# lazzati-astro/MCRaT

Measured on AMD Instinct MI355X. Metric: photon-scatter-events/sec at 1e6 photons, 2D FLASH jet, higher is better.
Workload: dtype f64

## Files before the change

mcrat_amd/csrc/frame_queue.hpp:

```cpp
#pragma once
#include <stddef.h>
#include <string.h>
#include "device_types.hpp"

#if defined(__HIPCC__)
#define MCRAT_FQ_HD __host__ __device__
#else
#define MCRAT_FQ_HD
#endif

namespace mcrat {

struct FrameItem {
    unsigned long long seed;
    double time_now;
    double remaining_time;
    double frame_end;
    int open;
    int hydro;
};
struct alignas(32) FrameRecord {
    double remaining_time, time_now;
    long long iterations;
    int done;
    int last_scattered_index;
    double last_time_step, last_scattered_temp;
    long long frame_scatt_cnt, n_relocated;
    long long not_found, kn_rejections, rescans, slot_steps;
    MCRAT_FQ_HD void from_state(const LoopState &s)
    {
        remaining_time = s.remaining_time; time_now = s.time_now; iterations = s.iterations; done = s.done; last_scattered_index = s.last_scattered_index;
        last_time_step = s.last_time_step; last_scattered_temp = s.last_scattered_temp; frame_scatt_cnt = s.frame_scatt_cnt; n_relocated = s.n_relocated;
        not_found = s.not_found; kn_rejections = s.kn_rejections; rescans = s.rescans; slot_steps = s.slot_steps;
    }
};
static_assert(sizeof(FrameRecord) <= 128, "the frame record stays compact: at most half a LoopState");
struct FrameQueueDev {
    int n_frames;
    int restore;
    int chain_clock;
    int pad;
    unsigned *ticket;
    const int *order;
    int order_off[9];
    unsigned *frames_done;
    const FrameItem *items;
    const HydroDev *hydro;
    FrameRecord *records;
    long long snap_delta;
    long long capture_delta, capture_stride;
};
constexpr unsigned FRAME_STALLED = 0x80000000u;
constexpr int FRAME_QUEUE_XCDS = 8, FRAME_TICKET_STRIDE = 16;


struct FrameQueueLayout {
    struct Range { size_t off, bytes; };
    size_t off_items, off_hydro, off_desc, off_ticket, off_done, off_rec, bytes;
    Range up;
    Range down;
    Range words;
    static size_t align_up(size_t x, size_t a) { return (x + a - 1) / a * a; }
    FrameQueueLayout(int R, int F, size_t n_hydro)
    {
        const size_t N = (size_t)R * (size_t)F;
        off_items = align_up(sizeof(int) * N, 64);
        off_hydro = align_up(off_items + sizeof(FrameItem) * N, 256);
        off_desc = align_up(off_hydro + sizeof(HydroDev) * n_hydro, 64);
        off_ticket = align_up(off_desc + sizeof(RankDesc) * (size_t)R, 256);
        off_done = off_ticket + sizeof(unsigned) * FRAME_QUEUE_XCDS * FRAME_TICKET_STRIDE;
        off_rec = align_up(off_done + sizeof(unsigned) * (size_t)R, 256);
        bytes = off_rec + sizeof(FrameRecord) * N;
        up = Range{0, off_rec};
        down = Range{off_ticket, bytes - off_ticket};
        words = Range{off_ticket, off_rec - off_ticket};
    }
    template <class T> static T *at(void *base, size_t off) { return reinterpret_cast<T *>(static_cast<char *>(base) + off); }
    int *order(void *b) const { return at<int>(b, 0); }
    FrameItem *items(void *b) const { return at<FrameItem>(b, off_items); }
    HydroDev *hydro(void *b) const { return at<HydroDev>(b, off_hydro); }
    RankDesc *desc(void *b) const { return at<RankDesc>(b, off_desc); }
    unsigned *ticket(void *b) const { return at<unsigned>(b, off_ticket); }
    unsigned *frames_done(void *b) const { return at<unsigned>(b, off_done); }
    FrameRecord *records(void *b) const { return at<FrameRecord>(b, off_rec); }
};

inline int frame_list_class(int r) { return r % FRAME_QUEUE_XCDS; }

inline int frame_queue_order(const FrameItem *items, int R, int F, const int *xcd_of_class, int *order, int *order_off)
{
    int count[FRAME_QUEUE_XCDS] = {0}, fill[FRAME_QUEUE_XCDS], n_open = 0, longest = 0;
    for (int f = 0; f < F; ++f)
        for (int r = 0; r < R; ++r)
            if (items[(size_t)f * R + r].open) count[xcd_of_class[frame_list_class(r)]] += 1;
    for (int x = 0; x < FRAME_QUEUE_XCDS; ++x) {
        order_off[x] = fill[x] = n_open;
        n_open += count[x];
        if (count[x] > longest) longest = count[x];
    }
    order_off[FRAME_QUEUE_XCDS] = n_open;
    for (int f = 0; f < F; ++f)
        for (int r = 0; r < R; ++r)
            if (items[(size_t)f * R + r].open) order[fill[xcd_of_class[frame_list_class(r)]]++] = f * R + r;
    return longest;
}
inline int frame_queue_groups(int longest_queue) { return FRAME_QUEUE_XCDS * longest_queue; }

enum FrameQueueNext { FRAME_QUEUE_DONE = 0, FRAME_QUEUE_GO_ON = 1, FRAME_QUEUE_NO_DRAW = 2 };
inline FrameQueueNext frame_queue_after_launch(unsigned *frames_done, unsigned *tickets, const FrameRecord *records, FrameItem *items, int R,
                                               const int *first, const int *last, bool chain_clock, int *stalled, int *xcd_of_class)
{
    bool all = true;
    for (int r = 0; r < R; ++r) {
        if (frames_done[r] & FRAME_STALLED) { frames_done[r] &= ~FRAME_STALLED; stalled[r] = (int)frames_done[r]; }
        all = all && (first[r] < 0 || (int)frames_done[r] == last[r] + 1);
    }
    if (all) return FRAME_QUEUE_DONE;
    int alive[FRAME_QUEUE_XCDS], n_alive = 0;
    for (int x = 0; x < FRAME_QUEUE_XCDS; ++x)
        if (tickets[(size_t)x * FRAME_TICKET_STRIDE] > 0) alive[n_alive++] = x;
    if (n_alive == 0) return FRAME_QUEUE_NO_DRAW;
    for (int k = 0; k < FRAME_QUEUE_XCDS; ++k)
        if (tickets[(size_t)xcd_of_class[k] * FRAME_TICKET_STRIDE] == 0) xcd_of_class[k] = alive[k % n_alive];
    memset(tickets, 0, sizeof(unsigned) * FRAME_QUEUE_XCDS * FRAME_TICKET_STRIDE);
    for (int r = 0; r < R; ++r) {
        if (first[r] < 0) continue;
        const int nf = (int)frames_done[r] > first[r] ? (int)frames_done[r] : first[r];
        for (int f = first[r]; f <= last[r]; ++f) {
            FrameItem &it = items[(size_t)f * R + r];
            if (f < nf) { it.open = 0; continue; }
            if (f > nf) continue;
            const FrameRecord &rec = records[(size_t)f * R + r];
            if (stalled[r] == nf && rec.iterations > 0 && !rec.done) it.open = 2;
            else if (chain_clock && f > first[r]) {
                it.time_now = records[(size_t)(f - 1) * R + r].time_now;
                it.remaining_time = it.frame_end - it.time_now;
// ... 8 lines not shown
```

mcrat_amd/csrc/kernels.hip:

```cpp
#include <hip/hip_runtime.h>
#include <limits.h>
#include <math.h>
#include <stdio.h>
#include <type_traits>
#include "device_types.hpp"
#include "launch.hpp"
#include "sc_exchange.hpp"
#include "physics.hpp"
#include "photon_cols.hpp"
#include "photon_plan.hpp"
#include "rng.hpp"
#include "cs_device.hpp"

#if !defined(MCRAT_TAU_TABLE_TU) || !defined(MCRAT_TU_DIMS)
#error "compile kernels.hip through kernels_d*.hip / kernels_table_d*.hip"
#endif
#define MCRAT_NS_CAT2(a, b) a##b
#define MCRAT_NS_CAT(a, b) MCRAT_NS_CAT2(a, b)
#if MCRAT_TAU_TABLE_TU
#define MCRAT_TU_NS MCRAT_NS_CAT(tau_table_d, MCRAT_TU_DIMS)
#else
#define MCRAT_TU_NS MCRAT_NS_CAT(tau_direct_d, MCRAT_TU_DIMS)
#endif

// ... 936 lines not shown
        if (nz && have + k == need - 1) *s_pos = q + 1;
        if (q >= n && have + k < need) *error = 1;
        __syncthreads();
        if (have + found >= need) { pos = *s_pos; have = need; }
        else { have += found; pos += BLOCK; }
        __syncthreads();
    }
    if (pos > n) { if (tid == 0) *error = 1; pos = n; }
    return pos;
}

__global__ __launch_bounds__(TAPE_BLOCK) void tape_draw_kernel(PhotonDev ph, const LoopState *__restrict__ st, TapeDev tape, Cand *__restrict__ block_min,
                                                                int n_blocks, Shortlist *sl)
{
    __shared__ double s_u[TAPE_BLOCK];
    __shared__ int s_w[TAPE_BLOCK / 64];
    __shared__ long long s_pos;
    __shared__ double s_wt[TAPE_BLOCK / 64];
    __shared__ int s_wi[TAPE_BLOCK / 64];
    if (st->done) return;
    const int tid = threadIdx.x;
    const double t_cut = st->t_cut;
    long long pos = *tape.cursor;
    if (tid == 0) sl->count = 0;
    __syncthreads();
    MinCand best;
    best.init();
    for (int c0 = 0; c0 < ph.n; c0 += TAPE_BLOCK) {
        const int i = c0 + tid;
        const bool valid = i < ph.n && (ph.flags[i] & FLAG_VALID);
        const bool located = valid && ph.idx[i] != -1;
        int need = 0;
        const int rank = block_exclusive_scan<TAPE_BLOCK>(located ? 1 : 0, s_w, need);
        pos = tape_take_nonzero<TAPE_BLOCK>(tape.u, tape.n, tape.error, pos, need, s_u, s_w, &s_pos);
        if (valid) {
            double t = ph.tts[i];
            if (located) {
                t = div_by_c(ph.ntau[i] * log(s_u[rank]));
                ph.tts[i] = t;
            }
            best.offer(t, i);
            if (t < t_cut) shortlist_push(sl, t, i);
        }
        __syncthreads();
    }
    wave_min_pair_dpp(best.t, best.i);
    if ((tid & 63) == 0) { s_wt[tid >> 6] = best.t; s_wi[tid >> 6] = best.i; }
    __syncthreads();
    if (tid == 0) {
        MinCand m;
        m.init();
        for (int w = 0; w < TAPE_BLOCK / 64; ++w) m.offer(s_wt[w], s_wi[w]);
        Cand c;
        c.t = m.t; c.idx = m.i; c.pad = 0;
        block_min[0] = c;
        *tape.cursor = pos;
    }
    for (int b = 1 + tid; b < n_blocks; b += TAPE_BLOCK) { Cand c; c.t = INFINITY; c.idx = INT_MAX; c.pad = 0; block_min[b] = c; }
}

__device__ __attribute__((noinline)) void copy_list_columns(double *r0, unsigned col_stride, int *idx, unsigned char *flags, char *type, int base, int n,
                                                            long long from, long long to, int tid, int block)
{
    for (int il = tid; il < n; il += block) {
        const size_t i = (size_t)base + il;
        double v[N_DOUBLE_COLS];
#pragma unroll
        for (int k = 0; k < N_DOUBLE_COLS; ++k)
            v[k] = *reinterpret_cast<const double *>(reinterpret_cast<const char *>(r0 + (size_t)k * col_stride + i) + from);
        const int ci = *reinterpret_cast<const int *>(reinterpret_cast<const char *>(idx + i) + from);
        const unsigned char cf = *reinterpret_cast<const unsigned char *>(reinterpret_cast<const char *>(flags + i) + from);
        const char ct = *(reinterpret_cast<const char *>(type + i) + from);
#pragma unroll
        for (int k = 0; k < N_DOUBLE_COLS; ++k)
            *reinterpret_cast<double *>(reinterpret_cast<char *>(r0 + (size_t)k * col_stride + i) + to) = v[k];
        *reinterpret_cast<int *>(reinterpret_cast<char *>(idx + i) + to) = ci;
        *reinterpret_cast<unsigned char *>(reinterpret_cast<char *>(flags + i) + to) = cf;
        *(reinterpret_cast<char *>(type + i) + to) = ct;
    }
}

template <unsigned MASK, int PITCH>
__device__ __attribute__((noinline)) void restore_list_columns_lds(double *r0, unsigned col_stride, int *idx, unsigned char *flags, char *type, int base,
                                                                   int n, long long from, unsigned char *lds, int tid, int block)
{
    using Cols = ListCols<MASK, PITCH>;
    static_assert((MASK & COLBIT_IDX) && (MASK & COLBIT_FLAGS), "idx and flags are among the LDS columns");
    typedef __attribute__((address_space(3))) unsigned char *LdsBytes;
    typedef __attribute__((address_space(3))) double *LdsDoubles;
    typedef __attribute__((address_space(3))) int *LdsInts;
    const LdsBytes l = (LdsBytes)lds;
    for (int il = tid; il < n; il += block) {
        const size_t i = (size_t)base + il;
        double v[N_DOUBLE_COLS];
#pragma unroll
        for (int k = 0; k < N_DOUBLE_COLS; ++k)
            v[k] = *reinterpret_cast<const double *>(reinterpret_cast<const char *>(r0 + (size_t)k * col_stride + i) + from);
        const int ci = *reinterpret_cast<const int *>(reinterpret_cast<const char *>(idx + i) + from);
        const unsigned char cf = *reinterpret_cast<const unsigned char *>(reinterpret_cast<const char *>(flags + i) + from);
        const char ct = *(reinterpret_cast<const char *>(type + i) + from);
#pragma unroll
        for (int k = 0; k < N_DOUBLE_COLS; ++k) {
            if (Cols::in_lds(k)) ((LdsDoubles)l)[Cols::lds_pos(k) * PITCH + il] = v[k];
            else r0[(size_t)k * col_stride + i] = v[k];
        }
        ((LdsInts)(l + Cols::lds_idx_bytes))[il] = ci;
        (l + Cols::lds_flags_bytes)[il] = cf;
        type[i] = ct;
    }
}

struct RankLayout {
    int n_ranks;
    int stride;
    int n_total;
    const RankDesc *desc;
    CsFrame *cs;
    const CsHookArgs *hook;
    FrameQueueDev fq;
};
struct TapeLayout : RankLayout {
    const double *tape_u;
    TapeList *tapes;
};
template <int BLOCK>
struct TapeLds {
    double u[BLOCK];
    int w[BLOCK / 64];
    long long pos, cursor;
};

#ifndef RANK_WAVES_PER_SIMD
#define RANK_WAVES_PER_SIMD 2
#endif
#ifndef RANK_NS_FUSED
#define RANK_NS_FUSED 2
#endif
#ifndef RANK_FUSE_DEN
#define RANK_FUSE_DEN 2
#endif

template <int DIMS, int GEOM, bool STOKES, bool RESIDENT, int RANK_BLOCK, bool FUSE, bool CSH = false, bool QUEUE = false, bool TAPE = false>
__global__ __launch_bounds__(RANK_BLOCK, RANK_WAVES_PER_SIMD) void rank_loop_kernel(PhotonDev gph, HydroDev hy_arg, LoopState *states, RngKey key,
                                                                std::conditional_t<TAPE, TapeLayout, RankLayout> lay, long long max_passes)
{
    constexpr int EVENT_BLOCK = RANK_BLOCK;
#ifndef RANK_NS_SPHERICAL
#define RANK_NS_SPHERICAL 4
#endif
    constexpr int RANK_NS_QUEUE = (GEOM == GEOM_SPHERICAL) ? RANK_NS_SPHERICAL : 4;
    constexpr int RANK_QCAP = 4 * RANK_BLOCK;
    extern __shared__ __align__(16) unsigned char s_dyn[];
    __shared__ LoopState st;
    __shared__ EventSharedT<RANK_BLOCK> sh;
    __shared__ int s_qn, s_sln, s_nrel, s_hook, s_len, s_item, s_ndefer;
    __shared__ int s_qb[RANK_QCAP];
    static_assert(sizeof(sh.list) >= sizeof(int) * RANK_QCAP, "queue fits into the sorted-list storage");
    int *const s_q = reinterpret_cast<int *>(sh.list);
    [[maybe_unused]] TapeLds<RANK_BLOCK> *tl = nullptr;
    if constexpr (TAPE) {
        __shared__ TapeLds<RANK_BLOCK> s_tape;
        tl = &s_tape;
    }
    int tid = threadIdx.x, lane = tid & 63;
    const bool queued = QUEUE ? lay.fq.n_frames > 0 : false;
    auto list_frame = [&](const int rank, const int item, const HydroDev &hy) __attribute__((always_inline)) {
    const int base = rank * lay.stride;
    int n = min(lay.stride, lay.n_total - base);
    RngKey rk = {key.seed, key.stream + (uint32_t)rank, 0u};
    if (lay.desc) {
        const RankDesc d = lay.desc[rank];
        n = min(n, d.len);
        rk.seed = d.seed;
        rk.stream = d.stream;
    }
    if (item >= 0) rk.seed = lay.fq.items[item].seed;
    const bool fresh = item >= 0 && lay.fq.items[item].open == 1;
    const int idx_shift = lay.desc ? base : 0;
    if (fresh) {
        static_assert(sizeof(LoopState) / sizeof(int) <= 64, "one wavefront clears the state");
        if (tid < (int)(sizeof(LoopState) / sizeof(int))) reinterpret_cast<int *>(&st)[tid] = 0;
        __syncthreads();
        if (tid == 0) {
            double t_now = lay.fq.items[item].time_now, rem = lay.fq.items[item].remaining_time;
            if (lay.fq.chain_clock && item >= lay.n_ranks && lay.fq.items[item - lay.n_ranks].open) {
                t_now = states[rank].time_now;
                rem = lay.fq.items[item].frame_end - t_now;
            }
            st.remaining_time = rem;
            st.time_now = t_now;
            st.done = !(rem > 0);
            st.skip_idx = -1;
            st.last_scattered_index = -1;
            st.force_relocate = 1;
        }
    } else if (tid == 0) {
        st = states[rank];
        if (st.last_scattered_index >= 0) st.last_scattered_index += idx_shift;
    }
    [[maybe_unused]] bool taped = false;
    [[maybe_unused]] TapeSource tsrc;
    if constexpr (TAPE) {
        const TapeList td = lay.tapes[rank];
        taped = td.n > 0;
        tsrc.t.u = lay.tape_u + td.offset; tsrc.t.n = td.n; tsrc.t.cursor = &tl->cursor; tsrc.t.error = &lay.tapes[rank].error;
        if (tid == 0) tl->cursor = td.cursor;
    }
    __syncthreads();
    if (st.done || n <= 0) {
        if (item >= 0 && tid == 0) { states[rank] = st; lay.fq.records[item].from_state(st); }
        if (fresh && n > 0) {
            if (lay.fq.restore) {
                copy_list_columns(gph.r0, gph.col_stride, gph.idx, gph.flags, gph.type, base, n, lay.fq.snap_delta, 0, tid, RANK_BLOCK);
                __syncthreads();
            }
            if (lay.fq.capture_delta != 0 && item / lay.n_ranks < lay.fq.n_frames - 1)
                copy_list_columns(gph.r0, gph.col_stride, gph.idx, gph.flags, gph.type, base, n, 0, lay.fq.capture_delta + (long long)(item / lay.n_ranks) * lay.fq.capture_stride, tid, RANK_BLOCK);
        }
        return;
    }
    [[maybe_unused]] bool lean_restored = false;
    if (fresh && lay.fq.restore) {
#ifndef MCRAT_NO_LEAN_RESTORE
        if constexpr (QUEUE && RESIDENT && RANK_BLOCK == 256) lean_restored = lay.cs == nullptr;
#endif
        if (lean_restored) {
            restore_list_columns_lds<LIST_MASK_FULL, rank_lds_limit(RANK_BLOCK)>(gph.r0, gph.col_stride, gph.idx, gph.flags, gph.type, base, n, lay.fq.snap_delta, s_dyn, tid, RANK_BLOCK);
        } else {
            copy_list_columns(gph.r0, gph.col_stride, gph.idx, gph.flags, gph.type, base, n, lay.fq.snap_delta, 0, tid, RANK_BLOCK);
            __syncthreads();
        }
    }
    int n_pass = n;
    auto settle_pass_limit = [&]() {
        int last = -1;
        for (int il = tid; il < n; il += EVENT_BLOCK) {
            const int i = base + il;
            const bool settled_null = gph.type[i] == 'N' && gph.idx[i] == -1 && gph.tts[i] == 1e12 / C_LIGHT;
            if (!settled_null) last = il;
        }
#pragma unroll
        for (int off = 32; off > 0; off >>= 1) last = max(last, __shfl_xor(last, off, 64));
        if (lane == 0) sh.wi[tid >> 6] = last;
        __syncthreads();
#pragma unroll
        for (int wv = 0; wv < EVENT_BLOCK / 64; ++wv) last = max(last, sh.wi[wv]);
        __syncthreads();
        n_pass = min(n, max(2, (last + 2) & ~1));
    };
    if (lay.cs) settle_pass_limit();
#ifdef MCRAT_DIAG
    long long dg[16] = {};
    long long dg_t = (long long)__builtin_amdgcn_s_memtime();
    const bool dg_clock = (g_diag & 1024) != 0;
    const long long dg_real0 = (long long)__builtin_amdgcn_s_memrealtime(), dg_tick0 = dg_t;
#define RANK_TICK(k) do { if (!dg_clock) { __builtin_amdgcn_sched_barrier(0); const long long n_ = (long long)__builtin_amdgcn_s_memtime(); dg[k] += n_ - dg_t; dg_t = n_; __builtin_amdgcn_sched_barrier(0); } } while (0)
#else
#define RANK_TICK(k) do { } while (0)
#endif

    constexpr bool FULL_HOT = RANK_BLOCK == 256;
    constexpr unsigned LDS_MASK = RESIDENT ? (FULL_HOT ? LIST_MASK_FULL : LIST_MASK_SMALL) : 0u;
    using Cols = ListCols<LDS_MASK, RESIDENT ? rank_lds_limit(RANK_BLOCK) : 0>;
    static_assert(Cols::lds_bytes_per_slot == (RESIDENT ? (size_t)rank_lds_bytes_per_slot(RANK_BLOCK) : 0), "rank_form_resolve sizes the dynamic LDS (lds_bytes) with this");
    const Cols ph(gph, RESIDENT ? s_dyn : nullptr, base);
    if constexpr (RESIDENT) {
        if (!lean_restored) {
            for (int il = tid; il < n; il += EVENT_BLOCK) {
                const int i = base + il;
                ph.r0(i) = ph.template gcol<COL_R0>(i); ph.r1(i) = ph.template gcol<COL_R1>(i); ph.r2(i) = ph.template gcol<COL_R2>(i);
                ph.ntau(i) = ph.template gcol<COL_NTAU>(i);
                if constexpr (FULL_HOT) {
                    ph.u0(i) = ph.template gcol<COL_U0>(i); ph.u1(i) = ph.template gcol<COL_U1>(i); ph.u2(i) = ph.template gcol<COL_U2>(i);
                    ph.idx(i) = ph.g_idx_at(i); ph.flags(i) = ph.g_flags_at(i);
                }
            }
            __syncthreads();
        }
    }
#ifndef MCRAT_NO_SHADOW_DRAWS
    constexpr bool SHADOW = RANK_BLOCK > 64 && !TAPE;
#else
    constexpr bool SHADOW = false;
#endif
    auto draw_logs = [&](unsigned long long it, int first_thread, int n_threads) {
        for (int pair = tid - first_thread; 2 * pair < n_pass; pair += n_threads) {
            const Philox4 blk = keyed_block(rk.seed, it, (uint32_t)pair, RNG_FREEPATH, rk.stream);
            const int i = base + 2 * pair;
            ph.draw_log(i) = log(bits_to_uniform_pos((uint64_t)blk.w[0] | ((uint64_t)blk.w[1] << 32)));
            if (2 * pair + 1 < n) ph.draw_log(i + 1) = log(bits_to_uniform_pos((uint64_t)blk.w[2] | ((uint64_t)blk.w[3] << 32)));
        }
    };
    if constexpr (SHADOW) {
        draw_logs(st.iteration, 0, EVENT_BLOCK);
        __syncthreads();
    } else {
        if (lean_restored) __syncthreads();
    }
    RANK_TICK(0);

    auto apply_pending = [&]() {
        const int nseg = st.nseg, skip = st.skip_idx;
        if (nseg > 0) {
            for (int il = tid; il < n; il += EVENT_BLOCK) {
                const int i = base + il;
                if ((ph.flags(i) & FLAG_MOVES) && i != skip) {
                    const double u0 = ph.u0(i), u1 = ph.u1(i), u2 = ph.u2(i);
                    double r0 = ph.r0(i), r1 = ph.r1(i), r2 = ph.r2(i);
                    for (int s = 0; s < nseg; ++s) {
                        const double t = st.seg[s];
                        r0 += u0 * t; r1 += u1 * t; r2 += u2 * t;
                    }
                    ph.r0(i) = r0; ph.r1(i) = r1; ph.r2(i) = r2;
                }
            }
        }
    };
    int prev_rel = 0;
    for (long long pass = 0; pass < max_passes; ++pass) {
        const int nseg = st.nseg;
        const int skip = st.skip_idx;
        const unsigned long long iter = st.iteration;
        const double t_cut = st.t_cut;
        const bool force = st.force_relocate != 0;
        const bool fused = FUSE && !TABLE_MODE && (force || RANK_FUSE_DEN * prev_rel > n_pass);
        if (tid == 0) { s_qn = 0; s_sln = 0; s_nrel = 0; s_ndefer = 0; }
        __syncthreads();
        if (!force) RANK_TICK(8);
        int n_rel = 0;

        MinCand best;
        best.init();
        int relocated = 0, not_found = 0;
        auto shortlist_lds = [&](double t, int i) {
            const int pos = atomicAdd(&s_sln, 1);
            if (pos < RANK_BLOCK) { sh.raw[pos].t = t; sh.raw[pos].idx = i; sh.raw[pos].pad = 0; }
        };
        for (int c0 = 0; c0 < n_pass; c0 += RANK_QCAP) {
            const int c1 = min(n_pass, c0 + RANK_QCAP);
            if (c0 > 0) {
                __syncthreads();
                if (tid == 0) { s_qn = 0; s_ndefer = 0; }
                __syncthreads();
            }
            auto phase1 = [&](auto ns_c, auto fused_c) {
                constexpr int NS = decltype(ns_c)::value;
                constexpr bool FUSED = decltype(fused_c)::value;
                constexpr int PAIRS = NS / 2;
                for (int pair = (c0 >> 1) + tid; 2 * pair < c1; pair += PAIRS * EVENT_BLOCK) {
                    int il[NS];
                    bool live[NS];
#pragma unroll
                    for (int j = 0; j < PAIRS; ++j) { il[2 * j] = 2 * (pair + j * EVENT_BLOCK); il[2 * j + 1] = il[2 * j] + 1; }
#pragma unroll
                    for (int k = 0; k < NS; ++k) { live[k] = il[k] < c1; if (!live[k]) il[k] = c0; }
                    double r0[NS], r1[NS], r2[NS], ntau[NS];
                    int cell[NS];
                    unsigned fl[NS];
#pragma unroll
                    for (int k = 0; k < NS; ++k) {
                        const int i = base + il[k];
                        r0[k] = ph.r0(i); r1[k] = ph.r1(i); r2[k] = ph.r2(i);
                        ntau[k] = ph.ntau(i); cell[k] = ph.idx(i); fl[k] = ph.flags(i);
                    }
                    if (nseg > 0) {
                        double u0[NS], u1[NS], u2[NS];
                        bool mv[NS];
#pragma unroll
                        for (int k = 0; k < NS; ++k) {
                            const int i = base + il[k];
                            u0[k] = ph.u0(i); u1[k] = ph.u1(i); u2[k] = ph.u2(i);
                            mv[k] = live[k] && (fl[k] & FLAG_MOVES) && (base + il[k] != skip);
                        }
                        for (int sg = 0; sg < nseg; ++sg) {
                            const double t = st.seg[sg];
#pragma unroll
                            for (int k = 0; k < NS; ++k) {
                                const double n0 = r0[k] + u0[k] * t, n1 = r1[k] + u1[k] * t, n2 = r2[k] + u2[k] * t;
                                r0[k] = mv[k] ? n0 : r0[k]; r1[k] = mv[k] ? n1 : r1[k]; r2[k] = mv[k] ? n2 : r2[k];
                            }
                        }
#pragma unroll
// ... 155 lines not shown
                    const int q = s_q[e];
                    const int i = base + (q & ~(Q_RECALC_ONLY | Q_DEFERRED));
                    if constexpr (TABLE_MODE) {
                        if (round == 1) {
                            if (!(q & Q_DEFERRED)) continue;
                            const double norm = phys::table_fallback_wave(ph.tau(i), ph.ntau(i), ts.seed, ts.pass, ts.slot_base + (uint32_t)(i - base), ts.stream,
                                                                          hy.hot_fallback_calls);
                            if (lane != 0) continue;
                            atomicAdd(hy.table_fallbacks, 1);
                            ts.mode = 2;
                            ts.norm = norm;
                        }
                    }
                    const uint64_t qbits = (uint64_t)__double_as_longlong(ph.tts(i));
                    const double t = slow_one<DIMS, GEOM, true>(ph, hy, i, !(q & Q_RECALC_ONLY), s_qb[e], !force, qbits, relocated, not_found, ts);
                    if constexpr (TABLE_MODE) {
                        if (ts.deferred) {
                            ts.deferred = false;
                            ph.tau(i) = ts.eps;
                            ph.ntau(i) = ts.theta;
                            s_q[e] = q | Q_DEFERRED;
                            s_ndefer = 1;
                            continue;
                        }
                    }
                    best.offer(t, i);
                    if (t < t_cut) shortlist_lds(t, i);
                }
            }
        }
        if constexpr (TAPE) {
            if (taped) {
                __syncthreads();
                if (tid == 0) s_sln = 0;
                best.init();
                long long pos = tl->cursor;
                __syncthreads();
                for (int c0 = 0; c0 < n_pass; c0 += RANK_BLOCK) {
                    const int i = base + c0 + tid;
                    const bool valid = c0 + tid < n_pass && (ph.flags(i) & FLAG_VALID);
                    const bool located = valid && ph.idx(i) != -1;
                    int need = 0;
                    const int k = block_exclusive_scan<RANK_BLOCK>(located ? 1 : 0, tl->w, need);
                    pos = tape_take_nonzero<RANK_BLOCK>(tsrc.t.u, tsrc.t.n, tsrc.t.error, pos, need, tl->u, tl->w, &tl->pos);
                    if (valid) {
                        double t = ph.tts(i);
                        if (located) {
                            t = div_by_c(ph.ntau(i) * log(tl->u[k]));
                            ph.tts(i) = t;
                        }
                        best.offer(t, i);
                        if (t < t_cut) shortlist_lds(t, i);
                    }
                    __syncthreads();
                }
                if (tid == 0) tl->cursor = pos;
            }
        }
        if (!force) RANK_TICK(9);
        wave_min_pair_dpp(best.t, best.i);
        if (lane == 0) { sh.wt[tid >> 6] = best.t; sh.wi[tid >> 6] = best.i; }
        if (!force) RANK_TICK(10);
        {
            const int w_rel = wave_sum_lane63_dpp(relocated), w_nf = wave_sum_lane63_dpp(not_found);
            if (lane == 63) {
                if (w_rel) atomicAdd(reinterpret_cast<unsigned long long *>(&st.n_relocated), (unsigned long long)w_rel);
                if (w_nf) atomicAdd(reinterpret_cast<unsigned long long *>(&st.not_found), (unsigned long long)w_nf);
            }
        }
        if (!force) RANK_TICK(11);
        __syncthreads();
        if (!force) RANK_TICK(12);
        prev_rel = s_nrel;
        MinCand g;
        g.init();
#pragma unroll
        for (int wv = 0; wv < EVENT_BLOCK / 64; ++wv) g.offer(sh.wt[wv], sh.wi[wv]);
        Cand gmin;
        gmin.t = g.t; gmin.idx = g.i; gmin.pad = 0;
        if (force) RANK_TICK(1); else RANK_TICK(13);
        const bool frame_goes_on = gmin.t < st.remaining_time;
        if constexpr (SHADOW) { if (frame_goes_on && tid >= 64) draw_logs(iter + 1, 64, RANK_BLOCK - 64); }
        (void)frame_goes_on;
        if constexpr (TAPE) {
            if (taped) event_block<DIMS, GEOM, STOKES, RANK_BLOCK>(ph, hy, &st, rk, sh, s_sln, gmin, base, n_pass, iter, st.remaining_time, st.last_scattered_index, st.t_est, tsrc);
            else event_block<DIMS, GEOM, STOKES, RANK_BLOCK>(ph, hy, &st, rk, sh, s_sln, gmin, base, n_pass, iter, st.remaining_time, st.last_scattered_index, st.t_est);
        } else {
            event_block<DIMS, GEOM, STOKES, RANK_BLOCK>(ph, hy, &st, rk, sh, s_sln, gmin, base, n_pass, iter, st.remaining_time, st.last_scattered_index, st.t_est);
        }
        if (tid == 0) {
            st.force_relocate = 0;
            s_hook = 0;
            if (lay.cs && st.photon_event_called) {
                const int sidx = st.last_scattered_index;
                const bool pool_photon = sidx >= 0 && gph.type[sidx] == 'p';
                const bool thousand = (st.frame_scatt_cnt % 1000 == 0) && st.frame_scatt_cnt != 0;
                if (pool_photon || thousand) {
                    if (CSH && lay.hook) {
                        s_hook = 1;
                    } else {
                        lay.cs[rank].halt = CS_HALT_HOOK;
                        lay.cs[rank].saved_done = st.done;
                        st.done = LOOP_CS_HALT;
                    }
                }
            }
        }
        __syncthreads();
        if constexpr (CSH) {
            if (s_hook) {
                apply_pending();
                __syncthreads();
                if (tid == 0) { st.nseg = 0; st.skip_idx = -1; s_len = n; }
                __syncthreads();
                PhotonDev lp = gph;
                offset_photons(lp, (size_t)base);
                lp.n = n;
                cs_hook_body<RANK_BLOCK>(lay.hook->p, hy, lay.hook->h, rk, &st, lp, &lay.cs[rank], 1, sh.wi, lay.stride, &s_len, idx_shift);
                __threadfence_block();
                __syncthreads();
                if (s_len != n) {
                    n = s_len;
                    if (tid == 0) const_cast<RankDesc *>(lay.desc)[rank].len = n;
                }
                settle_pass_limit();
                if constexpr (SHADOW) {
                    draw_logs(st.iteration, 0, EVENT_BLOCK);
                    __syncthreads();
                }
            }
        }
        RANK_TICK(3);
#ifdef MCRAT_DIAG
        dg[5] += 1;
        if (!force) dg[14] += 1;
#endif
        if (st.done) break;
    }

    {
        apply_pending();
        __syncthreads();
        if constexpr (RESIDENT) {
            for (int il = tid; il < n; il += EVENT_BLOCK) {
                const int i = base + il;
                ph.template gcol<COL_R0>(i) = ph.r0(i); ph.template gcol<COL_R1>(i) = ph.r1(i); ph.template gcol<COL_R2>(i) = ph.r2(i);
                ph.template gcol<COL_NTAU>(i) = ph.ntau(i);
                if constexpr (FULL_HOT) {
                    ph.template gcol<COL_U0>(i) = ph.u0(i); ph.template gcol<COL_U1>(i) = ph.u1(i); ph.template gcol<COL_U2>(i) = ph.u2(i);
                    ph.g_idx_at(i) = ph.idx(i); ph.g_flags_at(i) = ph.flags(i);
                }
            }
        }
#ifdef MCRAT_DIAG
        __syncthreads();
        RANK_TICK(4);
        dg[2] = dg[9] + dg[10] + dg[11] + dg[12] + dg[13];
        if (tid == 0) for (int k = 0; k < 8; ++k) st.stamps[k] = (g_diag & 2048) ? (k < 6 ? dg[8 + k] : dg[k == 6 ? 5 : 14]) : dg[k];
        if (tid == 0 && dg_clock) {
            st.stamps[0] = dg_real0; st.stamps[1] = (long long)__builtin_amdgcn_s_memrealtime();
            st.stamps[2] = (long long)__builtin_amdgcn_s_memtime() - dg_tick0;
        }
#endif
        if (tid == 0) {
            st.nseg = 0; st.skip_idx = -1;
            if (st.last_scattered_index >= 0) st.last_scattered_index -= idx_shift;
            states[rank] = st;
            if (item >= 0) lay.fq.records[item].from_state(st);
            if constexpr (TAPE) lay.tapes[rank].cursor = tl->cursor;
        }
        if (item >= 0 && lay.fq.capture_delta != 0 && item / lay.n_ranks < lay.fq.n_frames - 1 && st.done == LOOP_DONE) {
            __syncthreads();
            copy_list_columns(gph.r0, gph.col_stride, gph.idx, gph.flags, gph.type, base, n, 0, lay.fq.capture_delta + (long long)(item / lay.n_ranks) * lay.fq.capture_stride, tid, RANK_BLOCK);
        }
    }
    };

    for (;;) {
    if constexpr (QUEUE) { asm volatile("" : "+v"(tid)); lane = tid & 63; }
    int rank = blockIdx.x, item = -1;
    if (queued) {
        if (tid == 0) {
            unsigned xcc;
            asm volatile("s_getreg_b32 %0, hwreg(HW_REG_XCC_ID)" : "=s"(xcc));
            xcc &= (unsigned)(FRAME_QUEUE_XCDS - 1);
            const unsigned k = atomicAdd(lay.fq.ticket + xcc * FRAME_TICKET_STRIDE, 1u);
            int it = k < (unsigned)(lay.fq.order_off[xcc + 1] - lay.fq.order_off[xcc]) ? lay.fq.order[lay.fq.order_off[xcc] + (int)k] : -2;
            const int f = it / lay.n_ranks, r = it - f * lay.n_ranks;
            if (it >= 0 && f > 0 && lay.fq.items[it - lay.n_ranks].open) {
                unsigned d = 0;
                long long spins = 0;
                for (;;) {
                    d = __hip_atomic_load(&lay.fq.frames_done[r], __ATOMIC_RELAXED, __HIP_MEMORY_SCOPE_AGENT);
                    if (d >= (unsigned)f || spins >= (1ll << 22)) break;
                    __builtin_amdgcn_s_sleep(32);
                    spins += 1;
                }
                if (d != (unsigned)f) it = -1;
                __builtin_amdgcn_fence(__ATOMIC_ACQUIRE, "agent");
                asm volatile("s_waitcnt vmcnt(0)" ::: "memory");
            }
            s_item = it;
        }
        __syncthreads();
        item = __builtin_amdgcn_readfirstlane(s_item);
        if (item == -2) return;
        if (item < 0) { __syncthreads(); continue; }
        rank = item % lay.n_ranks;
    }
    if constexpr (QUEUE) {
        typedef const HydroDev __attribute__((address_space(4))) *ConstHydro;
        ConstHydro frames = (ConstHydro)lay.fq.hydro;
        const int h = __builtin_amdgcn_readfirstlane(lay.fq.items[item].hydro);
        list_frame(rank, item, *(const HydroDev *)(frames + h));
    } else {
        list_frame(rank, item, hy_arg);
    }
    if (queued) {
        asm volatile("s_waitcnt vmcnt(0)" ::: "memory");
        __syncthreads();
        if (tid == 0) {
            const unsigned frame = (unsigned)(item / lay.n_ranks);
            __hip_atomic_store(&lay.fq.frames_done[rank], st.done == LOOP_DONE ? frame + 1u : (FRAME_STALLED | frame), __ATOMIC_RELAXED, __HIP_MEMORY_SCOPE_AGENT);
        }
    }
    if (!(QUEUE && queued)) break;
    __syncthreads();
    }
}


#ifndef FAST_BLOCK_THREADS
#define FAST_BLOCK_THREADS 256
#endif
constexpr int FAST_BLOCK = FAST_BLOCK_THREADS;
constexpr uint32_t RNG_FAST_FREEPATH = 8u;

template <int DIMS, int GEOM, bool STOKES>
__global__ __launch_bounds__(FAST_BLOCK, 2) void fast_frame_kernel(PhotonDev ph, HydroDev hy, RngKey key, double remaining_time, int windows,
                                                                   int max_passes, FastCounts *__restrict__ counts, FastLists lists)
{
    __shared__ int s_q[2 * FAST_BLOCK];
    __shared__ int s_nq;
    __shared__ unsigned long long s_cnt[6];
#ifdef MCRAT_DIAG
    __shared__ LoopState s_stamps;
    LoopState *const stamp_state = &s_stamps;
#else
    LoopState *const stamp_state = nullptr;
#endif
    const int tid = threadIdx.x;
    const PtrCols pcols(ph);
    const int i0 = 2 * (blockIdx.x * FAST_BLOCK + tid);
    int first = 0, len = ph.n;
    if (lists.desc) {
        const int r = (2 * blockIdx.x * FAST_BLOCK) / lists.stride;
        const RankDesc d = lists.desc[r];
        first = r * lists.stride;
        len = d.len;
        remaining_time = lists.remaining_time[r];
        if (lists.windows) windows = lists.windows[r];
        if (len <= 0 || !(remaining_time > 0)) return;
        key.seed = d.seed; key.stream = d.stream; key.slot_base = 0;
        counts += r;
    }
    const uint32_t rng_first = key.slot_base - (uint32_t)first;
    const double window = remaining_time / (double)windows;
    double t_left[2], w_left[2];
    bool done[2], moves[2];
#pragma unroll
    for (int k = 0; k < 2; ++k) {
        const int i = i0 + k;
        const bool have = i - first < len && i < ph.n;
        const unsigned fl0 = have ? (unsigned)ph.flags[i] : 0u;
        moves[k] = (fl0 & FLAG_MOVES) != 0;
        t_left[k] = remaining_time; w_left[k] = window;
        done[k] = !(have && (fl0 & FLAG_VALID)) || !(remaining_time > 0);
    }
    int relocated = 0, not_found = 0;
    unsigned steps = 0, scatt = 0, rej = 0;
    if (tid < 6) s_cnt[tid] = 0;
    int pass = 0;
    for (; pass < max_passes; ++pass) {
        if (tid == 0) s_nq = 0;
        __syncthreads();
        if (!done[0] || !done[1]) {
            const int slot[2] = {i0, i0 + 1};
            unsigned fl[2];
            int cell[2], queue[2], code[2];
            double r0[2], r1[2], r2[2], a0[2], a1[2], a2[2], t[2];
            uint64_t bits[2];
            bool act[2];
#pragma unroll
            for (int k = 0; k < 2; ++k) {
                const int i = slot[k];
                act[k] = !done[k];
                if (!act[k]) {
                    fl[k] = 0; cell[k] = -1; queue[k] = 0; code[k] = -1; bits[k] = 0; t[k] = 0;
                    r0[k] = r1[k] = r2[k] = a0[k] = a1[k] = a2[k] = 0;
                    continue;
                }
                fl[k] = ph.flags[i];
// ... 577 lines not shown
```

mcrat_amd/csrc/rank_form_plan.hpp:

```cpp
#pragma once
#include <stddef.h>
#include "device_types.hpp"

namespace mcrat {

#ifndef RANK_SMALL
#define RANK_SMALL 128
#endif
constexpr int RANK_COLUMNS_GLOBAL = 1 << 30;

constexpr int rank_lds_bytes_per_slot(int block) { return block == 256 ? 7 * (int)sizeof(double) + (int)sizeof(int) + 1 : 4 * (int)sizeof(double); }
constexpr int rank_lds_limit(int block) { return block == 128 ? 1024 : (block == 512 ? 4096 : 1088); }
static_assert(2 * (13024 + rank_lds_limit(256) * rank_lds_bytes_per_slot(256)) <= 160 * 1024 &&
              4 * (6736 + rank_lds_limit(128) * rank_lds_bytes_per_slot(128)) <= 160 * 1024 &&
              25616 + rank_lds_limit(512) * rank_lds_bytes_per_slot(512) <= 160 * 1024, "the lists per CU of each form fit the CU's LDS at the full pitch");

constexpr bool rank_build_exists(int geom, bool table, bool resident, int threads, bool fuse, bool hook, bool queue, bool tape)
{
    if (tape) return threads == 256 && !resident && !fuse && !hook && !queue;
    if (hook) return (threads == 64 || threads == RANK_SMALL || threads == 256) && !resident && !fuse && !queue;
    if (fuse && (table || geom == GEOM_SPHERICAL || (threads != 256 && threads != 512))) return false;
    if (queue) return threads == 256 && resident;
    return threads == RANK_SMALL || threads == 256 || threads == 512;
}

struct RankForm { bool stokes, resident; int threads; bool fuse, hook, queue; };
struct RankFormRequest {
    int threads;
    bool fuse;
    bool hook;
    bool queued;
    int longest_list;
    bool stokes;
    int geometry;
    bool table;
    bool no_lds_lists;
};
struct RankFormPlan {
    RankForm form;
    int lds_slots;
    size_t dyn_bytes;
    bool no_queue_build;
    size_t lds_bytes;
};
inline RankFormPlan rank_form_resolve(const RankFormRequest &q)
{
    RankFormPlan p{RankForm{q.stokes, false, 256, false, q.hook, q.queued}, 0, 0, false, 0};
    const int block = (q.threads == 128 || (q.threads == 64 && q.hook) || (q.threads == 512 && !q.hook)) ? q.threads : 256;
    p.form.threads = block == 128 ? RANK_SMALL : block;
    if (!q.hook) {
        if (!q.no_lds_lists && q.longest_list <= rank_lds_limit(block)) p.lds_slots = (q.longest_list + 15) & ~15;
        p.form.resident = p.lds_slots > 0;
    }
    p.dyn_bytes = (size_t)p.lds_slots * rank_lds_bytes_per_slot(block);
    p.lds_bytes = p.form.resident ? (size_t)rank_lds_limit(p.form.threads) * rank_lds_bytes_per_slot(p.form.threads) : 0;
    p.form.fuse = q.fuse && rank_build_exists(q.geometry, q.table, p.form.resident, p.form.threads, true, q.hook, q.queued, false);
    p.no_queue_build = q.queued && !rank_build_exists(q.geometry, q.table, p.form.resident, p.form.threads, p.form.fuse, q.hook, true, false);
    return p;
}

inline int rank_queue_grid(int n_open, int per_cu, int cus) { return (per_cu > 0 && cus > 0 && per_cu * cus < n_open) ? per_cu * cus : n_open; }

struct RankBlock { int threads; bool fuse; };
struct RankEnv { bool block_set = false; int block = 0; bool fuse_set = false; int fuse = 0; };

inline RankBlock rank_block_rule(int n_ranks, int cus, int longest_list, double passes_per_list, int geometry, const RankEnv &env)
{
    RankBlock b;
    if (env.block_set) {
        b.threads = env.block == 128 ? 128 : (env.block == 512 ? 512 : 256);
        b.fuse = passes_per_list < 48.0;
    } else {
        const bool many = n_ranks > 2 * cus && longest_list <= 1024;
        const bool very_many = n_ranks >= 12 * cus && longest_list <= 1024;
        b.threads = ((many && passes_per_list >= 48.0) || very_many) ? 128 : 256;
        if (longest_list > 1088 && n_ranks <= cus + cus / 4) b.threads = 512;
        b.fuse = passes_per_list < 48.0 && geometry != GEOM_SPHERICAL;
    }
    if (env.fuse_set) b.fuse = env.fuse != 0;
    return b;
}

inline RankBlock cs_rank_block_rule(int n_ranks, int cus, bool hook_kernel, const RankEnv &env)
{
    RankBlock b{n_ranks > 2 * cus ? 128 : 256, false};
    if (n_ranks > 8 * cus && !hook_kernel) b.threads = 64;
    if (env.block_set) b.threads = env.block == 64 ? 64 : (env.block == 128 ? 128 : 256);
    return b;
}

}
```

Before: 22.45 million.

## Add queue lookahead: park next frame item and prefetch its restore and draws

```diff
diff --git a/mcrat_amd/csrc/frame_queue.hpp b/mcrat_amd/csrc/frame_queue.hpp
--- a/mcrat_amd/csrc/frame_queue.hpp
+++ b/mcrat_amd/csrc/frame_queue.hpp
@@ -52,6 +52,21 @@
 };
 constexpr unsigned FRAME_STALLED = 0x80000000u;
 constexpr int FRAME_QUEUE_XCDS = 8, FRAME_TICKET_STRIDE = 16;
+
+struct alignas(16) ParkedItem {
+    int item;
+    int valid;
+    int pred_open;
+    int rank;
+    int start_pass;
+    int chunks;
+    int n;
+    int pad;
+    RankDesc desc;
+    FrameItem fi;
+};
+constexpr int FRAME_AHEAD_SLOTS = 192;
+static_assert(sizeof(ParkedItem) == 96, "the parked item stays small: two lists per CU leave 1.2 KB of LDS free");
 
 
 struct FrameQueueLayout {
diff --git a/mcrat_amd/csrc/kernels.hip b/mcrat_amd/csrc/kernels.hip
--- a/mcrat_amd/csrc/kernels.hip
+++ b/mcrat_amd/csrc/kernels.hip
@@ -1042,7 +1042,7 @@
 
 template <unsigned MASK, int PITCH>
 __device__ __attribute__((noinline)) void restore_list_columns_lds(double *r0, unsigned col_stride, int *idx, unsigned char *flags, char *type, int base,
-                                                                   int n, long long from, unsigned char *lds, int tid, int block)
+                                                                   int n, long long from, unsigned char *lds, int tid, int block, int global_from = 0)
 {
     using Cols = ListCols<MASK, PITCH>;
     static_assert((MASK & COLBIT_IDX) && (MASK & COLBIT_FLAGS), "idx and flags are among the LDS columns");
@@ -1050,7 +1050,21 @@
     typedef __attribute__((address_space(3))) double *LdsDoubles;
     typedef __attribute__((address_space(3))) int *LdsInts;
     const LdsBytes l = (LdsBytes)lds;
-    for (int il = tid; il < n; il += block) {
+    int il = tid;
+    for (; il < min(n, global_from); il += block) {
+        const size_t i = (size_t)base + il;
+        double v[Cols::n_lds_doubles];
+#pragma unroll
+        for (int k = 0; k < N_DOUBLE_COLS; ++k)
+            if (Cols::in_lds(k)) v[Cols::lds_pos(k)] = *reinterpret_cast<const double *>(reinterpret_cast<const char *>(r0 + (size_t)k * col_stride + i) + from);
+        const int ci = *reinterpret_cast<const int *>(reinterpret_cast<const char *>(idx + i) + from);
+        const unsigned char cf = *reinterpret_cast<const unsigned char *>(reinterpret_cast<const char *>(flags + i) + from);
+#pragma unroll
+        for (int p = 0; p < Cols::n_lds_doubles; ++p) ((LdsDoubles)l)[p * PITCH + il] = v[p];
+        ((LdsInts)(l + Cols::lds_idx_bytes))[il] = ci;
+        (l + Cols::lds_flags_bytes)[il] = cf;
+    }
+    for (; il < n; il += block) {
         const size_t i = (size_t)base + il;
         double v[N_DOUBLE_COLS];
 #pragma unroll
@@ -1068,6 +1082,94 @@
         (l + Cols::lds_flags_bytes)[il] = cf;
         type[i] = ct;
     }
+}
+
+__device__ __attribute__((noinline)) void frame_queue_draw(unsigned *ticket, const int *order, int count, const FrameItem *items, const RankDesc *desc,
+                                                           int n_ranks, int list_stride, int n_total, ParkedItem *out)
+{
+    const unsigned k = atomicAdd(ticket, 1u);
+    const int it = k < (unsigned)count ? order[k] : -2;
+    int pred_open = 0, rank = 0, n = 0;
+    if (it >= 0) {
+        const int f = it / n_ranks, r = it - f * n_ranks;
+        const FrameItem fi = items[it];
+        if (f > 0) pred_open = items[it - n_ranks].open != 0;
+        n = min(list_stride, n_total - r * list_stride);
+        if (desc) {
+            const RankDesc d = desc[r];
+            n = min(n, d.len);
+            out->desc = d;
+        }
+        out->fi = fi;
+        rank = r;
+    }
+    out->item = it;
+    out->pred_open = pred_open;
+    out->rank = rank;
+    out->n = n;
+    out->start_pass = -1;
+    out->chunks = 0;
+}
+
+template <unsigned MASK>
+__device__ __attribute__((noinline)) void frame_queue_prefetch(ParkedItem *park, double *r0, unsigned col_stride, char *type, int list_stride,
+                                                               long long snap_delta, bool draws, const unsigned *frames_done, int n_ranks,
+                                                               int running_rank, int pass, int t)
+{
+    if (!park->valid) return;
+    const int sp = park->start_pass;
+    if (sp == -1 && t == 0) {
+        const int it = park->item;
+        int go = -2;
+        if (it >= 0 && park->fi.open == 1 && park->rank != running_rank) {
+            if (!park->pred_open) {
+                go = pass + 1;
+            } else {
+                const unsigned d = __hip_atomic_load(&frames_done[park->rank], __ATOMIC_RELAXED, __HIP_MEMORY_SCOPE_AGENT);
+                const unsigned f = (unsigned)(it / n_ranks);
+                if (d == f) {
+                    __builtin_amdgcn_fence(__ATOMIC_ACQUIRE, "agent");
+                    go = pass + 1;
+                } else if (d < f) {
+                    go = -1;
+                }
+            }
+        }
+        park->start_pass = go;
+    }
+    if (sp < 0 || pass < sp) return;
+    const int n = park->n;
+    const int il = (pass - sp) * FRAME_AHEAD_SLOTS + t;
+    const int base = park->rank * list_stride;
+    if (snap_delta != 0 && il < n) {
+        const size_t i = (size_t)base + il;
+        const char ct = *(reinterpret_cast<const char *>(type + i) + snap_delta);
+#pragma unroll
+        for (int half = 0; half < 2; ++half) {
+            double v[N_DOUBLE_COLS / 2];
+#pragma unroll
+            for (int k = 0; k < N_DOUBLE_COLS / 2; ++k)
+                if (!((MASK >> (half * (N_DOUBLE_COLS / 2) + k)) & 1u))
+                    v[k] = *reinterpret_cast<const double *>(reinterpret_cast<const char *>(r0 + (size_t)(half * (N_DOUBLE_COLS / 2) + k) * col_stride + i) + snap_delta);
+#pragma unroll
+            for (int k = 0; k < N_DOUBLE_COLS / 2; ++k)
+                if (!((MASK >> (half * (N_DOUBLE_COLS / 2) + k)) & 1u)) r0[(size_t)(half * (N_DOUBLE_COLS / 2) + k) * col_stride + i] = v[k];
+        }
+        type[i] = ct;
+    }
+    const int pair = (pass - sp) * (FRAME_AHEAD_SLOTS / 2) + (t - FRAME_AHEAD_SLOTS / 2);
+    if (draws && t >= FRAME_AHEAD_SLOTS / 2 && 2 * pair < n) {
+        double *const draw_log = r0 + (size_t)N_DOUBLE_COLS * col_stride + (size_t)base;
+        const Philox4 blk = keyed_block(park->fi.seed, 0ull, (uint32_t)pair, RNG_FREEPATH, park->desc.stream);
+        draw_log[2 * pair] = log(bits_to_uniform_pos((uint64_t)blk.w[0] | ((uint64_t)blk.w[1] << 32)));
+        if (2 * pair + 1 < n) draw_log[2 * pair + 1] = log(bits_to_uniform_pos((uint64_t)blk.w[2] | ((uint64_t)blk.w[3] << 32)));
+    }
+}
+__device__ __forceinline__ int lds_uniform(int v) { return __builtin_amdgcn_readfirstlane(v); }
+__device__ __forceinline__ unsigned long long lds_uniform(unsigned long long v)
+{
+    const unsigned lo = (unsigned)__builtin_amdgcn_readfirstlane((int)(unsigned)v), hi = (unsigned)__builtin_amdgcn_readfirstlane((int)(unsigned)(v >> 32));
+    return ((unsigned long long)hi << 32) | lo;
 }
 
 struct RankLayout {
@@ -1122,30 +1224,107 @@
         __shared__ TapeLds<RANK_BLOCK> s_tape;
         tl = &s_tape;
     }
+#ifndef MCRAT_NO_QUEUE_LOOKAHEAD
+    constexpr bool LOOKAHEAD = QUEUE && !CSH && RANK_BLOCK > 64;
+#else
+    constexpr bool LOOKAHEAD = false;
+#endif
+    [[maybe_unused]] ParkedItem *park = nullptr;
+    if constexpr (LOOKAHEAD) {
+        static_assert(sizeof(ParkedItem) <= RANK_QUEUE_PARK_BYTES, "rank_form_plan.hpp holds two lists per CU against this");
+        __shared__ ParkedItem s_park;
+        park = &s_park;
+    }
+#ifdef MCRAT_DIAG
+    __shared__ long long s_qdg[5];
+#define QUEUE_STAMP(k) do { if (QUEUE && tid == 0) { __builtin_amdgcn_sched_barrier(0); s_qdg[k] = (long long)__builtin_amdgcn_s_memtime(); __builtin_amdgcn_sched_barrier(0); } } while (0)
+#else
+#define QUEUE_STAMP(k) do { } while (0)
+#endif
     int tid = threadIdx.x, lane = tid & 63;
     const bool queued = QUEUE ? lay.fq.n_frames > 0 : false;
+    [[maybe_unused]] auto draw_item = [&](const bool ahead) __attribute__((always_inline)) {
+        if constexpr (LOOKAHEAD) {
+            unsigned xcc;
+            asm volatile("s_getreg_b32 %0, hwreg(HW_REG_XCC_ID)" : "=s"(xcc));
+            xcc &= (unsigned)(FRAME_QUEUE_XCDS - 1);
+            unsigned *const ticket = lay.fq.ticket + xcc * FRAME_TICKET_STRIDE;
+            const int off = lay.fq.order_off[xcc], count = lay.fq.order_off[xcc + 1] - off;
+            if (ahead) {
+                const unsigned drawn = __hip_atomic_load(ticket, __ATOMIC_RELAXED, __HIP_MEMORY_SCOPE_AGENT);
+                if (drawn >= (unsigned)count || count - (int)drawn <= (int)(gridDim.x / FRAME_QUEUE_XCDS)) return false;
+            }
+            frame_queue_draw(ticket, lay.fq.order + off, count, lay.fq.items, lay.desc, lay.n_ranks, lay.stride, lay.n_total, park);
+            return true;
+        } else {
+            return false;
+        }
+    };
+    [[maybe_unused]] auto park_next = [&]() __attribute__((always_inline)) {
+        if constexpr (LOOKAHEAD) { if (draw_item(true)) park->valid = 1; }
+    };
+#ifndef MCRAT_QUEUE_LOOKAHEAD_PARTS
+#define MCRAT_QUEUE_LOOKAHEAD_PARTS 3
+#endif
+#ifndef MCRAT_NO_LEAN_RESTORE
+    constexpr bool AHEAD_RESTORE = LOOKAHEAD && RESIDENT && RANK_BLOCK == 256 && (MCRAT_QUEUE_LOOKAHEAD_PARTS & 1) != 0;
+#else
+    constexpr bool AHEAD_RESTORE = false;
+#endif
+#ifndef MCRAT_NO_SHADOW_DRAWS
+    constexpr bool AHEAD_DRAWS = LOOKAHEAD && RANK_BLOCK > 64 && !TAPE && (MCRAT_QUEUE_LOOKAHEAD_PARTS & 2) != 0;
+#else
+    constexpr bool AHEAD_DRAWS = false;
+#endif
+    [[maybe_unused]] auto prefetch_next = [&](const int running_rank, const int pass) __attribute__((always_inline)) {
+        if constexpr (AHEAD_RESTORE || AHEAD_DRAWS) {
+            if (lay.cs == nullptr && lay.desc != nullptr && tid - 64 < FRAME_AHEAD_SLOTS)
+                frame_queue_prefetch<LIST_MASK_FULL>(park, gph.r0, gph.col_stride, gph.type, lay.stride, AHEAD_RESTORE && lay.fq.restore ? lay.fq.snap_delta : 0ll,
+                                                     AHEAD_DRAWS, lay.fq.frames_done, lay.n_ranks, running_rank, pass, tid - 64);
+        }
+    };
     auto list_frame = [&](const int rank, const int item, const HydroDev &hy) __attribute__((always_inline)) {
     const int base = rank * lay.stride;
     int n = min(lay.stride, lay.n_total - base);
     RngKey rk = {key.seed, key.stream + (uint32_t)rank, 0u};
+    [[maybe_unused]] const bool parked = LOOKAHEAD && item >= 0;
+    bool fresh;
     if (lay.desc) {
-        const RankDesc d = lay.desc[rank];
+        RankDesc d;
+        if (parked) { d.len = lds_uniform(park->desc.len); d.stream = (uint32_t)lds_uniform((int)park->desc.stream); d.seed = lds_uniform((unsigned long long)park->desc.seed); }
+        else d = lay.desc[rank];
         n = min(n, d.len);
         rk.seed = d.seed;
         rk.stream = d.stream;
     }
-    if (item >= 0) rk.seed = lay.fq.items[item].seed;
-    const bool fresh = item >= 0 && lay.fq.items[item].open == 1;
+    if (parked) {
+        rk.seed = lds_uniform((unsigned long long)park->fi.seed);
+        fresh = lds_uniform(park->fi.open) == 1;
+    } else {
+        if (item >= 0) rk.seed = lay.fq.items[item].seed;
+        fresh = item >= 0 && lay.fq.items[item].open == 1;
+    }
+    [[maybe_unused]] int ahead_slots = 0;
+    if constexpr (AHEAD_RESTORE || AHEAD_DRAWS) { if (parked) ahead_slots = lds_uniform(park->chunks) * FRAME_AHEAD_SLOTS; }
     const int idx_shift = lay.desc ? base : 0;
     if (fresh) {
         static_assert(sizeof(LoopState) / sizeof(int) <= 64, "one wavefront clears the state");
         if (tid < (int)(sizeof(LoopState) / sizeof(int))) reinterpret_cast<int *>(&st)[tid] = 0;
         __syncthreads();
         if (tid == 0) {
-            double t_now = lay.fq.items[item].time_now, rem = lay.fq.items[item].remaining_time;
-            if (lay.fq.chain_clock && item >= lay.n_ranks && lay.fq.items[item - lay.n_ranks].open) {
-                t_now = states[rank].time_now;
-                rem = lay.fq.items[item].frame_end - t_now;
+            double t_now, rem;
+            if (parked) {
+                t_now = park->fi.time_now; rem = park->fi.remaining_time;
+                if (lay.fq.chain_clock && park->pred_open) {
+                    t_now = states[rank].time_now;
+                    rem = park->fi.frame_end - t_now;
+                }
+            } else {
+                t_now = lay.fq.items[item].time_now; rem = lay.fq.items[item].remaining_time;
+                if (lay.fq.chain_clock && item >= lay.n_ranks && lay.fq.items[item - lay.n_ranks].open) {
+                    t_now = states[rank].time_now;
+                    rem = lay.fq.items[item].frame_end - t_now;
+                }
             }
             st.remaining_time = rem;
             st.time_now = t_now;
@@ -1185,12 +1364,14 @@
         if constexpr (QUEUE && RESIDENT && RANK_BLOCK == 256) lean_restored = lay.cs == nullptr;
 #endif
         if (lean_restored) {
-            restore_list_columns_lds<LIST_MASK_FULL, rank_lds_limit(RANK_BLOCK)>(gph.r0, gph.col_stride, gph.idx, gph.flags, gph.type, base, n, lay.fq.snap_delta, s_dyn, tid, RANK_BLOCK);
+            restore_list_columns_lds<LIST_MASK_FULL, rank_lds_limit(RANK_BLOCK)>(gph.r0, gph.col_stride, gph.idx, gph.flags, gph.type, base, n, lay.fq.snap_delta, s_dyn, tid, RANK_BLOCK,
+                                                                                 AHEAD_RESTORE ? ahead_slots : 0);
         } else {
             copy_list_columns(gph.r0, gph.col_stride, gph.idx, gph.flags, gph.type, base, n, lay.fq.snap_delta, 0, tid, RANK_BLOCK);
             __syncthreads();
         }
     }
+    QUEUE_STAMP(3);
     int n_pass = n;
     auto settle_pass_limit = [&]() {
         int last = -1;
@@ -1243,8 +1424,8 @@
 #else
     constexpr bool SHADOW = false;
 #endif
-    auto draw_logs = [&](unsigned long long it, int first_thread, int n_threads) {
-        for (int pair = tid - first_thread; 2 * pair < n_pass; pair += n_threads) {
+    auto draw_logs = [&](unsigned long long it, int first_thread, int n_threads, int first_pair = 0) {
+        for (int pair = first_pair + tid - first_thread; 2 * pair < n_pass; pair += n_threads) {
             const Philox4 blk = keyed_block(rk.seed, it, (uint32_t)pair, RNG_FREEPATH, rk.stream);
             const int i = base + 2 * pair;
             ph.draw_log(i) = log(bits_to_uniform_pos((uint64_t)blk.w[0] | ((uint64_t)blk.w[1] << 32)));
@@ -1252,12 +1433,14 @@
         }
     };
     if constexpr (SHADOW) {
-        draw_logs(st.iteration, 0, EVENT_BLOCK);
+        if constexpr (AHEAD_DRAWS) draw_logs(st.iteration, 0, EVENT_BLOCK, ahead_slots / 2);
+        else draw_logs(st.iteration, 0, EVENT_BLOCK);
         __syncthreads();
     } else {
         if (lean_restored) __syncthreads();
     }
     RANK_TICK(0);
+    QUEUE_STAMP(4);
 
     auto apply_pending = [&]() {
         const int nseg = st.nseg, skip = st.skip_idx;
@@ -1579,6 +1762,12 @@
         const bool frame_goes_on = gmin.t < st.remaining_time;
         if constexpr (SHADOW) { if (frame_goes_on && tid >= 64) draw_logs(iter + 1, 64, RANK_BLOCK - 64); }
         (void)frame_goes_on;
+        if constexpr (LOOKAHEAD) {
+            if (item >= 0 && tid >= 64) {
+                if (pass == 0) { if (tid == 64) park_next(); }
+                else prefetch_next(rank, (int)pass);
+            }
+        }
         if constexpr (TAPE) {
             if (taped) event_block<DIMS, GEOM, STOKES, RANK_BLOCK>(ph, hy, &st, rk, sh, s_sln, gmin, base, n_pass, iter, st.remaining_time, st.last_scattered_index, st.t_est, tsrc);
             else event_block<DIMS, GEOM, STOKES, RANK_BLOCK>(ph, hy, &st, rk, sh, s_sln, gmin, base, n_pass, iter, st.remaining_time, st.last_scattered_index, st.t_est);
@@ -1586,6 +1775,9 @@
             event_block<DIMS, GEOM, STOKES, RANK_BLOCK>(ph, hy, &st, rk, sh, s_sln, gmin, base, n_pass, iter, st.remaining_time, st.last_scattered_index, st.t_est);
         }
         if (tid == 0) {
+            if constexpr (AHEAD_RESTORE || AHEAD_DRAWS) {
+                if (item >= 0 && pass > 0 && park->valid && park->start_pass >= 0 && pass >= park->start_pass) park->chunks += 1;
+            }
             st.force_relocate = 0;
             s_hook = 0;
             if (lay.cs && st.photon_event_called) {
@@ -1658,6 +1850,17 @@
             st.stamps[0] = dg_real0; st.stamps[1] = (long long)__builtin_amdgcn_s_memrealtime();
             st.stamps[2] = (long long)__builtin_amdgcn_s_memtime() - dg_tick0;
         }
+        if (QUEUE && tid == 0 && (g_diag & 4096)) {
+            if (item >= lay.n_ranks && item / lay.n_ranks == lay.fq.n_frames - 1) {
+                for (int k = 0; k < 8; ++k) st.stamps[k] = __hip_atomic_load(&states[rank].stamps[k], __ATOMIC_RELAXED, __HIP_MEMORY_SCOPE_AGENT);
+            } else {
+                for (int k = 0; k < 4; ++k) st.stamps[k] = s_qdg[k + 1] - s_qdg[k];
+                st.stamps[4] = s_qdg[0] != 0;
+                st.stamps[5] = (long long)__builtin_amdgcn_s_memtime() - s_qdg[4];
+                st.stamps[6] = dg[5];
+                st.stamps[7] = ahead_slots;
+            }
+        }
 #endif
         if (tid == 0) {
             st.nseg = 0; st.skip_idx = -1;
@@ -1673,18 +1876,35 @@
     }
     };
 
+    if constexpr (LOOKAHEAD) { if (tid == 0) park->valid = 0; }
+#ifdef MCRAT_DIAG
+    if (tid == 0) s_qdg[0] = 0;
+#endif
     for (;;) {
     if constexpr (QUEUE) { asm volatile("" : "+v"(tid)); lane = tid & 63; }
     int rank = blockIdx.x, item = -1;
     if (queued) {
         if (tid == 0) {
+            int it, f, r;
+            bool wait;
+            if constexpr (LOOKAHEAD) {
+                if (park->valid) park->valid = 0;
+                else draw_item(false);
+                QUEUE_STAMP(1);
+                it = park->item;
+                f = it / lay.n_ranks; r = it - f * lay.n_ranks;
+                wait = it >= 0 && park->pred_open != 0;
+            } else {
             unsigned xcc;
             asm volatile("s_getreg_b32 %0, hwreg(HW_REG_XCC_ID)" : "=s"(xcc));
             xcc &= (unsigned)(FRAME_QUEUE_XCDS - 1);
             const unsigned k = atomicAdd(lay.fq.ticket + xcc * FRAME_TICKET_STRIDE, 1u);
-            int it = k < (unsigned)(lay.fq.order_off[xcc + 1] - lay.fq.order_off[xcc]) ? lay.fq.order[lay.fq.order_off[xcc] + (int)k] : -2;
-            const int f = it / lay.n_ranks, r = it - f * lay.n_ranks;
-            if (it >= 0 && f > 0 && lay.fq.items[it - lay.n_ranks].open) {
+            it = k < (unsigned)(lay.fq.order_off[xcc + 1] - lay.fq.order_off[xcc]) ? lay.fq.order[lay.fq.order_off[xcc] + (int)k] : -2;
+            QUEUE_STAMP(1);
+            f = it / lay.n_ranks; r = it - f * lay.n_ranks;
+            wait = it >= 0 && f > 0 && lay.fq.items[it - lay.n_ranks].open;
+            }
+            if (wait) {
                 unsigned d = 0;
                 long long spins = 0;
                 for (;;) {
@@ -1700,6 +1920,7 @@
             s_item = it;
         }
         __syncthreads();
+        QUEUE_STAMP(2);
         item = __builtin_amdgcn_readfirstlane(s_item);
         if (item == -2) return;
         if (item < 0) { __syncthreads(); continue; }
@@ -1708,13 +1929,16 @@
     if constexpr (QUEUE) {
         typedef const HydroDev __attribute__((address_space(4))) *ConstHydro;
         ConstHydro frames = (ConstHydro)lay.fq.hydro;
-        const int h = __builtin_amdgcn_readfirstlane(lay.fq.items[item].hydro);
+        int h;
+        if constexpr (LOOKAHEAD) h = __builtin_amdgcn_readfirstlane(item >= 0 ? park->fi.hydro : lay.fq.items[item].hydro);
+        else h = __builtin_amdgcn_readfirstlane(lay.fq.items[item].hydro);
         list_frame(rank, item, *(const HydroDev *)(frames + h));
     } else {
         list_frame(rank, item, hy_arg);
     }
     if (queued) {
         asm volatile("s_waitcnt vmcnt(0)" ::: "memory");
+        QUEUE_STAMP(0);
         __syncthreads();
         if (tid == 0) {
             const unsigned frame = (unsigned)(item / lay.n_ranks);
diff --git a/mcrat_amd/csrc/rank_form_plan.hpp b/mcrat_amd/csrc/rank_form_plan.hpp
--- a/mcrat_amd/csrc/rank_form_plan.hpp
+++ b/mcrat_amd/csrc/rank_form_plan.hpp
@@ -11,7 +11,8 @@
 
 constexpr int rank_lds_bytes_per_slot(int block) { return block == 256 ? 7 * (int)sizeof(double) + (int)sizeof(int) + 1 : 4 * (int)sizeof(double); }
 constexpr int rank_lds_limit(int block) { return block == 128 ? 1024 : (block == 512 ? 4096 : 1088); }
-static_assert(2 * (13024 + rank_lds_limit(256) * rank_lds_bytes_per_slot(256)) <= 160 * 1024 &&
+constexpr int RANK_QUEUE_PARK_BYTES = 96;
+static_assert(2 * (13024 + RANK_QUEUE_PARK_BYTES + rank_lds_limit(256) * rank_lds_bytes_per_slot(256)) <= 160 * 1024 &&
               4 * (6736 + rank_lds_limit(128) * rank_lds_bytes_per_slot(128)) <= 160 * 1024 &&
               25616 + rank_lds_limit(512) * rank_lds_bytes_per_slot(512) <= 160 * 1024, "the lists per CU of each form fit the CU's LDS at the full pitch");
 
```

Result: no change. 22.67 million (median of 6 runs) (+1.0%).
